# zakuro-ai/asr

Hardware: AMD Instinct MI355X
Metric: utterances/sec (10 s, 161-bin) DS2 5x1024 BiGRU CTC train step (higher is better)
Workload: dtype bf16

## Files before the change

### asr_amd/csrc/gemm_nt_w4.h

```cpp
constexpr int W4_LDS = 4 * G_TILE;
typedef __bf16 bf16x4w __attribute__((ext_vector_type(4)));
typedef float f32x2w __attribute__((ext_vector_type(2)));

__device__ __forceinline__ void w4_dma(unsigned voff, const char* sbase, unsigned lds_dst) {
  asm volatile("s_mov_b32 m0, %2\n\ts_nop 0\n\tglobal_load_lds_dwordx4 %0, %1" ::"v"(voff), "s"(sbase), "s"(lds_dst) : "memory");
}

template <bool OBF = false>
__global__ __launch_bounds__(256) void gemm_bf16_nt_w4_kernel(BArgs g, int ntx, int nty) {
  extern __shared__ __attribute__((aligned(1024))) char ldsg[];
  const int nt = ntx * nty;
  int orig = blockIdx.x;
  const int SR = g.super_rows > 0 ? g.super_rows : 1 << 20;
  auto tile_origin = [&](int o, int& tm0, int& tn0) {
    const int xcd = o & 7, q8 = nt >> 3, r8 = nt & 7;
    const int t = (xcd < r8 ? xcd * (q8 + 1) : r8 * (q8 + 1) + (xcd - r8) * q8) + (o >> 3);
    const int per = SR * ntx, sr = t / per, rem = t - sr * per;
    const int rows = min(SR, nty - sr * SR);
    const int tn = rem / rows;
    tm0 = (sr * SR + rem - tn * rows) * 256; tn0 = tn * 256;
  };
  int m0, n0;
  tile_origin(orig, m0, n0);
  const int nkt = g.K >> 6;
  const int lane = threadIdx.x & 63;
  const int wave = __builtin_amdgcn_readfirstlane(threadIdx.x >> 6);
  const int wm = wave >> 1, wn = wave & 1;
  const unsigned lds0 = (unsigned)(uintptr_t)(lds_void*)ldsg;

  unsigned voffA[8], voffB[8];
  const char* sA;
  const char* sB;
  auto retarget = [&](int tm0, int tn0) {
    int rl = lane;
    asm volatile("" : "+v"(rl));
    const int prow = rl >> 3;
#pragma unroll
    for (int p = 0; p < 8; ++p) {
      const int r = (wave + 4 * p) * 8 + prow;
      const int seg = (rl & 7) ^ ((r >> 1) & 7);
      voffA[p] = (unsigned)(min(r, g.M - 1 - tm0) * g.lda * 2 + seg * 16);
      voffB[p] = (unsigned)(min(r, g.N - 1 - tn0) * g.ldb * 2 + seg * 16);
    }
    sA = reinterpret_cast<const char*>(g.A + (long long)tm0 * g.lda);
    sB = reinterpret_cast<const char*>(g.B + (long long)tn0 * g.ldb);
  };
  retarget(m0, n0);
  const unsigned dstw = lds0 + wave * 1024;
  auto dma_a = [&](unsigned boff, int p) { w4_dma(voffA[p], sA, dstw + boff + p * 4096); };
  auto dma_b = [&](unsigned boff, int p) { w4_dma(voffB[p], sB, dstw + boff + 32768 + p * 4096); };

  const int frow = lane & 15, fseg = lane >> 4;
  const unsigned swz0 = (unsigned)((fseg ^ ((frow >> 1) & 7)) << 4);
  const unsigned raA0 = lds0 + (wm * 128 + frow) * 128 + swz0;
  const unsigned raB0 = lds0 + 32768 + (wn * 128 + frow) * 128 + swz0;

  f32x4 acc[8][8];
  f32x4 fa[2][8], fb[2][8];
#define W4_BC(x) __builtin_bit_cast(bf16x8, x)
#define W4_SB() __builtin_amdgcn_sched_barrier(0)
#define W4_RD(dst, addr, off) asm volatile("ds_read_b128 %0, %1 offset:%2" : "=v"(dst) : "v"(addr), "n"(off))
#define W4_LGKM0(F)                                                                                                                   \
  asm volatile("s_waitcnt lgkmcnt(0)"                                                                                                 \
               : "+v"(F[0]), "+v"(F[1]), "+v"(F[2]), "+v"(F[3]), "+v"(F[4]), "+v"(F[5]), "+v"(F[6]), "+v"(F[7])                       \
               :                                                                                                                      \
               : "memory")
#define W4_KTILE(DMA, VMW, NEXT)                                                                                                      \
  do {                                                                                                                                \
    const unsigned cA1 = (raA0 ^ 64u) + boff, cB1 = (raB0 ^ 64u) + boff, nA0 = raA0 + (boff ^ 65536u), nB0 = raB0 + (boff ^ 65536u);  \
    W4_SB();                                                                                                                          \
    _Pragma("unroll") for (int m_ = 0; m_ < 64; ++m_) {                                                                               \
      acc[m_ & 7][m_ >> 3] = __builtin_amdgcn_mfma_f32_16x16x32_bf16(W4_BC(fb[0][m_ >> 3]), W4_BC(fa[0][m_ & 7]), acc[m_ & 7][m_ >> 3], 0, 0, 0); \
      W4_SB();                                                                                                                        \
      if (m_ < 16 && !(m_ & 1)) W4_RD(fa[1][(m_ >> 1) & 7], cA1, ((m_ >> 1) & 7) * 2048);                                             \
      if (m_ == 19) W4_LGKM0(fa[1]);                                                                                                  \
      if (m_ == 20) __builtin_amdgcn_s_barrier();                                                                                     \
      if (m_ >= 21 && m_ <= 51 && (m_ & 1)) {                                                                                         \
        if (((m_ - 21) >> 1) & 1) W4_RD(fb[1][((m_ - 21) >> 2) & 7], cB1, (((m_ - 21) >> 2) & 7) * 2048);                             \
        else if (DMA) dma_a(boff, ((m_ - 21) >> 2) & 7);                                                                              \
      }                                                                                                                               \
      if (m_ == 54) W4_LGKM0(fb[1]);                                                                                                  \
      if (m_ == 55) __builtin_amdgcn_s_barrier();                                                                                     \
      if ((DMA) && (m_ == 57 || m_ == 59 || m_ == 61)) dma_b(boff, (m_ - 57) >> 1);                                                   \
      W4_SB();                                                                                                                        \
    }                                                                                                                                 \
    _Pragma("unroll") for (int m_ = 0; m_ < 64; ++m_) {                                                                               \
      acc[m_ & 7][m_ >> 3] = __builtin_amdgcn_mfma_f32_16x16x32_bf16(W4_BC(fb[1][m_ >> 3]), W4_BC(fa[1][m_ & 7]), acc[m_ & 7][m_ >> 3], 0, 0, 0); \
      W4_SB();                                                                                                                        \
      if ((DMA) && m_ < 10 && !(m_ & 1)) dma_b(boff, 3 + (m_ >> 1));                                                                  \
      if ((DMA) && m_ == 9) { sA += 128; sB += 128; }                                                                                 \
      if ((NEXT) && m_ == 10) asm volatile(VMW ::: "memory");                                                                         \
      if ((NEXT) && m_ == 11) __builtin_amdgcn_s_barrier();                                                                           \
      if ((NEXT) && m_ >= 13 && m_ <= 58 && (m_ - 13) % 3 == 0) {                                                                     \
        if ((m_ - 13) / 3 < 8) W4_RD(fa[0][((m_ - 13) / 3) & 7], nA0, (((m_ - 13) / 3) & 7) * 2048);                                  \
        else W4_RD(fb[0][((m_ - 13) / 3 - 8) & 7], nB0, (((m_ - 13) / 3 - 8) & 7) * 2048);                                            \
      }                                                                                                                               \
      W4_SB();                                                                                                                        \
    }                                                                                                                                 \
    if (NEXT) { W4_LGKM0(fa[0]); W4_LGKM0(fb[0]); }                                                                                   \
    W4_SB();                                                                                                                          \
    boff ^= 65536u;                                                                                                                   \
  } while (0)

  auto stage_first_two = [&]() {
#pragma unroll
    for (int p = 0; p < 8; ++p) { dma_a(0u, p); dma_b(0u, p); }
    sA += 128; sB += 128;
#pragma unroll
    for (int p = 0; p < 8; ++p) { dma_a(65536u, p); dma_b(65536u, p); }
    sA += 128; sB += 128;
  };
  stage_first_two();
  bool after_epilogue = false;
  for (;;) {
    if (after_epilogue) asm volatile("s_waitcnt vmcnt(63)" ::: "memory");
    else asm volatile("s_waitcnt vmcnt(0)" ::: "memory");
    __builtin_amdgcn_s_barrier();
    W4_SB();
#pragma unroll
    for (int i = 0; i < 8; ++i) W4_RD(fa[0][i], raA0, i * 2048);
#pragma unroll
    for (int j = 0; j < 8; ++j) W4_RD(fb[0][j], raB0, j * 2048);
#pragma unroll
    for (int i = 0; i < 8; ++i)
#pragma unroll
      for (int j = 0; j < 8; ++j) acc[i][j] = f32x4{0.f, 0.f, 0.f, 0.f};
    W4_LGKM0(fa[0]);
    W4_LGKM0(fb[0]);
    unsigned boff = 0u;
    int kt = 0;
    if (nkt > 2) {
      W4_KTILE(1, "", 1);
      kt = 1;
    }
    for (; kt < nkt - 2; ++kt) W4_KTILE(1, "s_waitcnt vmcnt(16)", 1);
    if (kt < nkt - 1) W4_KTILE(0, "s_waitcnt vmcnt(0)", 1);
    const bool more = orig + (int)gridDim.x < nt;
    int m0n = 0, n0n = 0;
    if (more) {
      tile_origin(orig + (int)gridDim.x, m0n, n0n);
      retarget(m0n, n0n);
    }
    f32x4 pbv[8];
#pragma unroll
    for (int j = 0; j < 8; ++j) {
      const int col = n0 + wn * 128 + j * 16 + fseg * 4;
      const char* bp = (g.bias && col < g.N) ? reinterpret_cast<const char*>(g.bias + col) : reinterpret_cast<const char*>(g_zero16);
      asm volatile("global_load_dwordx4 %0, %1, off" : "=v"(pbv[j]) : "v"(bp) : "memory");
    }
    W4_KTILE(0, "", 0);
    asm volatile("s_waitcnt vmcnt(0)"
                 : "+v"(pbv[0]), "+v"(pbv[1]), "+v"(pbv[2]), "+v"(pbv[3]), "+v"(pbv[4]), "+v"(pbv[5]), "+v"(pbv[6]), "+v"(pbv[7])
                 :
                 : "memory");
    if (more) stage_first_two();
    {
      float* C = g.C;
      const long long ldc = g.ldc;
      const bool stream_out = (g.nt_store & 1) != 0;
      int el = lane;
      asm volatile("" : "+v"(el));
      const int frow = el & 15, fseg = el >> 4;
      if constexpr (OBF) {
        __bf16* Cb = reinterpret_cast<__bf16*>(C);
#pragma unroll
        for (int i = 0; i < 8; ++i) {
          const int row = m0 + wm * 128 + i * 16 + frow;
#pragma unroll
          for (int j = 0; j < 8; j += 2) {
            const f32x4 va = acc[i][j] + pbv[j], vb = acc[i][j + 1] + pbv[j + 1];
            const bf16x4w pa = {(__bf16)va[0], (__bf16)va[1], (__bf16)va[2], (__bf16)va[3]};
            const bf16x4w pb = {(__bf16)vb[0], (__bf16)vb[1], (__bf16)vb[2], (__bf16)vb[3]};
            const f32x2w a2 = __builtin_bit_cast(f32x2w, pa), b2 = __builtin_bit_cast(f32x2w, pb);
            const u32pair s0 = permlane16_swap(a2[0], b2[0]), s1 = permlane16_swap(a2[1], b2[1]);
            const int col = n0 + wn * 128 + (j + (fseg & 1)) * 16 + (fseg >> 1) * 8;
            const f32x4 v = {s0.a, s1.a, s0.b, s1.b};
            f32x4* pc = (row < g.M && col < g.N) ? reinterpret_cast<f32x4*>(Cb + (long long)row * ldc + col) : reinterpret_cast<f32x4*>(g_sink16);
            if (stream_out) __builtin_nontemporal_store(v, pc);
            else *pc = v;
          }
        }
      } else
#pragma unroll
      for (int i = 0; i < 8; ++i) {
        const int row = m0 + wm * 128 + i * 16 + frow;
#pragma unroll
        for (int j = 0; j < 8; ++j) {
          const int col = n0 + wn * 128 + j * 16 + fseg * 4;
          const f32x4 v = acc[i][j] + pbv[j];
          f32x4* pc = (row < g.M && col < g.N) ? reinterpret_cast<f32x4*>(C + (long long)row * ldc + col) : reinterpret_cast<f32x4*>(g_sink16);
          if (stream_out) __builtin_nontemporal_store(v, pc);
          else *pc = v;
        }
      }
    }
    if (!more) break;
    orig += (int)gridDim.x; m0 = m0n; n0 = n0n;
    after_epilogue = true;
  }
  asm volatile("s_waitcnt vmcnt(0)" ::: "memory");
#undef W4_BC
#undef W4_SB
#undef W4_RD
#undef W4_LGKM0
#undef W4_KTILE
}
```

Measured before the change: 2828.

## Overlap previous tile's epilogue stores with next tile's first MFMA k-step

Restructures the persistent GEMM loop so the next tile's DMA staging happens continuously across tile boundaries, and the previous tile's accumulator stores (bias add plus nontemporal global stores) are interleaved into the first k-tile's MFMA stream as a 'seam' drain. Accumulators move to AGPRs via inline-asm MFMA, with a zero-C form for the first k-step, which removes explicit zeroing. Retargeting skips recomputing clamped offsets for interior tiles. The aim is to hide the epilogue store latency and the pipeline refill bubble between tiles. The cost is heavy reliance on hand-tuned waitcnt values and exec masking, which is fragile to get right.

```diff
diff --git a/asr_amd/csrc/gemm_nt_w4.h b/asr_amd/csrc/gemm_nt_w4.h
--- a/asr_amd/csrc/gemm_nt_w4.h
+++ b/asr_amd/csrc/gemm_nt_w4.h
@@ -31,16 +31,22 @@
   unsigned voffA[8], voffB[8];
   const char* sA;
   const char* sB;
+  bool clampA = true, clampB = true;
   auto retarget = [&](int tm0, int tn0) {
-    int rl = lane;
-    asm volatile("" : "+v"(rl));
-    const int prow = rl >> 3;
-#pragma unroll
-    for (int p = 0; p < 8; ++p) {
-      const int r = (wave + 4 * p) * 8 + prow;
-      const int seg = (rl & 7) ^ ((r >> 1) & 7);
-      voffA[p] = (unsigned)(min(r, g.M - 1 - tm0) * g.lda * 2 + seg * 16);
-      voffB[p] = (unsigned)(min(r, g.N - 1 - tn0) * g.ldb * 2 + seg * 16);
+    const bool eA = tm0 + 256 > g.M, eB = tn0 + 256 > g.N;
+    if (eA || clampA || eB || clampB) {
+      int rl = lane;
+      asm volatile("" : "+v"(rl));
+      const int prow = rl >> 3;
+      const int capA = (eA || clampA) ? g.M - 1 - tm0 : 255, capB = (eB || clampB) ? g.N - 1 - tn0 : 255;
+#pragma unroll
+      for (int p = 0; p < 8; ++p) {
+        const int r = (wave + 4 * p) * 8 + prow;
+        const int seg = (rl & 7) ^ ((r >> 1) & 7);
+        voffA[p] = (unsigned)(min(r, capA) * g.lda * 2 + seg * 16);
+        voffB[p] = (unsigned)(min(r, capB) * g.ldb * 2 + seg * 16);
+      }
+      clampA = eA; clampB = eB;
     }
     sA = reinterpret_cast<const char*>(g.A + (long long)tm0 * g.lda);
     sB = reinterpret_cast<const char*>(g.B + (long long)tn0 * g.ldb);
@@ -57,7 +63,6 @@
 
   f32x4 acc[8][8];
   f32x4 fa[2][8], fb[2][8];
-#define W4_BC(x) __builtin_bit_cast(bf16x8, x)
 #define W4_SB() __builtin_amdgcn_sched_barrier(0)
 #define W4_RD(dst, addr, off) asm volatile("ds_read_b128 %0, %1 offset:%2" : "=v"(dst) : "v"(addr), "n"(off))
 #define W4_LGKM0(F)                                                                                                                   \
@@ -65,30 +70,47 @@
                : "+v"(F[0]), "+v"(F[1]), "+v"(F[2]), "+v"(F[3]), "+v"(F[4]), "+v"(F[5]), "+v"(F[6]), "+v"(F[7])                       \
                :                                                                                                                      \
                : "memory")
-#define W4_KTILE(DMA, VMW, NEXT)                                                                                                      \
+#define W4_MFMA(c, b, a) asm volatile("v_mfma_f32_16x16x32_bf16 %0, %1, %2, %0" : "+a"(c) : "v"(b), "v"(a))
+#define W4_MFMA0(c, b, a) asm volatile("v_mfma_f32_16x16x32_bf16 %0, %1, %2, 0" : "+a"(c) : "v"(b), "v"(a))
+#define W4_MFMA_DONE() asm volatile("s_nop 15\n\ts_nop 7" ::: "memory")
+#define W4_ST(voff, data, sbase, imm, on)                                                                                        \
+  asm volatile("s_mov_b32 exec_lo, %4\n\ts_mov_b32 exec_hi, %4\n\tglobal_store_dwordx4 %0, %1, %2 offset:%3 nt\n\ts_mov_b64 exec, -1" \
+               ::"v"(voff), "v"(data), "s"(sbase), "n"(imm), "s"(on)                                                             \
+               : "memory")
+#define W4_KTILE(FIRST, DRAIN, VMA, VMW, NEXT)                                                                                        \
   do {                                                                                                                                \
     const unsigned cA1 = (raA0 ^ 64u) + boff, cB1 = (raB0 ^ 64u) + boff, nA0 = raA0 + (boff ^ 65536u), nB0 = raB0 + (boff ^ 65536u);  \
+    f32x4 dr_ = f32x4{0.f, 0.f, 0.f, 0.f};                                                                                            \
+    unsigned co_ = cvoff;                                                                                                             \
+    if (DRAIN) { dr_ = acc[0][0]; asm volatile("" : "+v"(dr_)); }                                                                     \
     W4_SB();                                                                                                                          \
     _Pragma("unroll") for (int m_ = 0; m_ < 64; ++m_) {                                                                               \
-      acc[m_ & 7][m_ >> 3] = __builtin_amdgcn_mfma_f32_16x16x32_bf16(W4_BC(fb[0][m_ >> 3]), W4_BC(fa[0][m_ & 7]), acc[m_ & 7][m_ >> 3], 0, 0, 0); \
-      W4_SB();                                                                                                                        \
+      if (FIRST) W4_MFMA0(acc[m_ & 7][m_ >> 3], fb[0][m_ >> 3], fa[0][m_ & 7]);                                                       \
+      else W4_MFMA(acc[m_ & 7][m_ >> 3], fb[0][m_ >> 3], fa[0][m_ & 7]);                                                              \
+      W4_SB();                                                                                                                        \
+      if (DRAIN) {                                                                                                                    \
+        const f32x4 v_ = dr_ + pbv[m_ >> 3];                                                                                          \
+        W4_ST(co_, v_, cbase, (m_ >> 3) * 64, con);                                                                                   \
+        co_ = (m_ & 7) == 7 ? cvoff : co_ + cstep;                                                                                    \
+        if (m_ < 63) { dr_ = acc[(m_ + 1) & 7][(m_ + 1) >> 3]; asm volatile("" : "+v"(dr_)); }                                        \
+      }                                                                                                                               \
       if (m_ < 16 && !(m_ & 1)) W4_RD(fa[1][(m_ >> 1) & 7], cA1, ((m_ >> 1) & 7) * 2048);                                             \
-      if (m_ == 19) W4_LGKM0(fa[1]);                                                                                                  \
+      if (m_ == 19) { asm volatile(VMA ::: "memory"); W4_LGKM0(fa[1]); }                                                              \
       if (m_ == 20) __builtin_amdgcn_s_barrier();                                                                                     \
       if (m_ >= 21 && m_ <= 51 && (m_ & 1)) {                                                                                         \
         if (((m_ - 21) >> 1) & 1) W4_RD(fb[1][((m_ - 21) >> 2) & 7], cB1, (((m_ - 21) >> 2) & 7) * 2048);                             \
-        else if (DMA) dma_a(boff, ((m_ - 21) >> 2) & 7);                                                                              \
+        else dma_a(boff, ((m_ - 21) >> 2) & 7);                                                                                       \
       }                                                                                                                               \
       if (m_ == 54) W4_LGKM0(fb[1]);                                                                                                  \
       if (m_ == 55) __builtin_amdgcn_s_barrier();                                                                                     \
-      if ((DMA) && (m_ == 57 || m_ == 59 || m_ == 61)) dma_b(boff, (m_ - 57) >> 1);                                                   \
+      if (m_ == 57 || m_ == 59 || m_ == 61) dma_b(boff, (m_ - 57) >> 1);                                                              \
       W4_SB();                                                                                                                        \
     }                                                                                                                                 \
     _Pragma("unroll") for (int m_ = 0; m_ < 64; ++m_) {                                                                               \
-      acc[m_ & 7][m_ >> 3] = __builtin_amdgcn_mfma_f32_16x16x32_bf16(W4_BC(fb[1][m_ >> 3]), W4_BC(fa[1][m_ & 7]), acc[m_ & 7][m_ >> 3], 0, 0, 0); \
-      W4_SB();                                                                                                                        \
-      if ((DMA) && m_ < 10 && !(m_ & 1)) dma_b(boff, 3 + (m_ >> 1));                                                                  \
-      if ((DMA) && m_ == 9) { sA += 128; sB += 128; }                                                                                 \
+      W4_MFMA(acc[m_ & 7][m_ >> 3], fb[1][m_ >> 3], fa[1][m_ & 7]);                                                                   \
+      W4_SB();                                                                                                                        \
+      if (m_ < 10 && !(m_ & 1)) dma_b(boff, 3 + (m_ >> 1));                                                                           \
+      if (m_ == 9) { sA += 128; sB += 128; }                                                                                          \
       if ((NEXT) && m_ == 10) asm volatile(VMW ::: "memory");                                                                         \
       if ((NEXT) && m_ == 11) __builtin_amdgcn_s_barrier();                                                                           \
       if ((NEXT) && m_ >= 13 && m_ <= 58 && (m_ - 13) % 3 == 0) {                                                                     \
@@ -102,62 +124,78 @@
     boff ^= 65536u;                                                                                                                   \
   } while (0)
 
-  auto stage_first_two = [&]() {
-#pragma unroll
-    for (int p = 0; p < 8; ++p) { dma_a(0u, p); dma_b(0u, p); }
-    sA += 128; sB += 128;
-#pragma unroll
-    for (int p = 0; p < 8; ++p) { dma_a(65536u, p); dma_b(65536u, p); }
-    sA += 128; sB += 128;
+#pragma unroll
+  for (int p = 0; p < 8; ++p) { dma_a(0u, p); dma_b(0u, p); }
+  sA += 128; sB += 128;
+#pragma unroll
+  for (int p = 0; p < 8; ++p) { dma_a(65536u, p); dma_b(65536u, p); }
+  sA += 128; sB += 128;
+  asm volatile("s_waitcnt vmcnt(0)" ::: "memory");
+#pragma unroll
+  for (int i = 0; i < 8; ++i)
+#pragma unroll
+    for (int j = 0; j < 8; ++j) asm volatile("" : "=a"(acc[i][j]));
+  unsigned boff = 0u;
+
+  const bool stream_out = (g.nt_store & 1) != 0;
+  bool more = false;
+  int m0n = 0, n0n = 0;
+  auto stage_next_tile = [&]() {
+    more = orig + (int)gridDim.x < nt;
+    m0n = m0; n0n = n0;
+    if (more) tile_origin(orig + (int)gridDim.x, m0n, n0n);
+    retarget(m0n, n0n);
   };
-  stage_first_two();
-  bool after_epilogue = false;
+  bool drain = false;
+  int mo = 0, no = 0;
+  f32x4 pbv[8] = {};
+  unsigned cvoff = 0u, cstep = 0u;
+  const char* cbase = nullptr;
+  int con = 0;
   for (;;) {
-    if (after_epilogue) asm volatile("s_waitcnt vmcnt(63)" ::: "memory");
-    else asm volatile("s_waitcnt vmcnt(0)" ::: "memory");
     __builtin_amdgcn_s_barrier();
     W4_SB();
 #pragma unroll
-    for (int i = 0; i < 8; ++i) W4_RD(fa[0][i], raA0, i * 2048);
-#pragma unroll
-    for (int j = 0; j < 8; ++j) W4_RD(fb[0][j], raB0, j * 2048);
-#pragma unroll
-    for (int i = 0; i < 8; ++i)
-#pragma unroll
-      for (int j = 0; j < 8; ++j) acc[i][j] = f32x4{0.f, 0.f, 0.f, 0.f};
+    for (int i = 0; i < 8; ++i) W4_RD(fa[0][i], raA0 + boff, i * 2048);
+#pragma unroll
+    for (int j = 0; j < 8; ++j) W4_RD(fb[0][j], raB0 + boff, j * 2048);
     W4_LGKM0(fa[0]);
     W4_LGKM0(fb[0]);
-    unsigned boff = 0u;
-    int kt = 0;
-    if (nkt > 2) {
-      W4_KTILE(1, "", 1);
-      kt = 1;
-    }
-    for (; kt < nkt - 2; ++kt) W4_KTILE(1, "s_waitcnt vmcnt(16)", 1);
-    if (kt < nkt - 1) W4_KTILE(0, "s_waitcnt vmcnt(0)", 1);
-    const bool more = orig + (int)gridDim.x < nt;
-    int m0n = 0, n0n = 0;
-    if (more) {
-      tile_origin(orig + (int)gridDim.x, m0n, n0n);
-      retarget(m0n, n0n);
-    }
-    f32x4 pbv[8];
+    W4_SB();
+    if (nkt == 2) stage_next_tile();
+    if constexpr (OBF) {
+      W4_KTILE(1, 0, "", "", 1);
+    } else {
+      if (drain) {
+        int el = lane;
+        asm volatile("" : "+v"(el));
+        cvoff = (unsigned)(((el & 15) * g.ldc + (el >> 4) * 4) * 4);
+        cstep = (unsigned)(g.ldc * 64);
+        cbase = reinterpret_cast<const char*>(g.C + (long long)(mo + wm * 128) * g.ldc + no + wn * 128);
+      }
+      con = __builtin_amdgcn_readfirstlane(drain ? -1 : 0);
+      W4_KTILE(1, 1, "s_waitcnt vmcnt(20)", "", 1);
+    }
+    for (int kt = 1; kt < nkt - 1; ++kt) {
+      if (kt == nkt - 2) stage_next_tile();
+      W4_KTILE(0, 0, "", "s_waitcnt vmcnt(16)", 1);
+    }
+    const bool seam = !OBF && more && stream_out && m0 + 256 <= g.M && n0 + 256 <= g.N && g.ldc < (1 << 22);
 #pragma unroll
     for (int j = 0; j < 8; ++j) {
       const int col = n0 + wn * 128 + j * 16 + fseg * 4;
       const char* bp = (g.bias && col < g.N) ? reinterpret_cast<const char*>(g.bias + col) : reinterpret_cast<const char*>(g_zero16);
       asm volatile("global_load_dwordx4 %0, %1, off" : "=v"(pbv[j]) : "v"(bp) : "memory");
     }
-    W4_KTILE(0, "", 0);
-    asm volatile("s_waitcnt vmcnt(0)"
+    W4_KTILE(0, 0, "", "", 0);
+    W4_MFMA_DONE();
+    asm volatile("s_waitcnt vmcnt(16)"
                  : "+v"(pbv[0]), "+v"(pbv[1]), "+v"(pbv[2]), "+v"(pbv[3]), "+v"(pbv[4]), "+v"(pbv[5]), "+v"(pbv[6]), "+v"(pbv[7])
                  :
                  : "memory");
-    if (more) stage_first_two();
-    {
+    if (!seam) {
       float* C = g.C;
       const long long ldc = g.ldc;
-      const bool stream_out = (g.nt_store & 1) != 0;
       int el = lane;
       asm volatile("" : "+v"(el));
       const int frow = el & 15, fseg = el >> 4;
@@ -179,6 +217,7 @@
             if (stream_out) __builtin_nontemporal_store(v, pc);
             else *pc = v;
           }
+          W4_SB();
         }
       } else
 #pragma unroll
@@ -187,19 +226,27 @@
 #pragma unroll
         for (int j = 0; j < 8; ++j) {
           const int col = n0 + wn * 128 + j * 16 + fseg * 4;
-          const f32x4 v = acc[i][j] + pbv[j];
+          f32x4 t = acc[i][j];
+          asm volatile("" : "+v"(t));
+          const f32x4 v = t + pbv[j];
           f32x4* pc = (row < g.M && col < g.N) ? reinterpret_cast<f32x4*>(C + (long long)row * ldc + col) : reinterpret_cast<f32x4*>(g_sink16);
           if (stream_out) __builtin_nontemporal_store(v, pc);
           else *pc = v;
         }
+        W4_SB();
       }
+      if constexpr (OBF) asm volatile("s_waitcnt vmcnt(32)" ::: "memory");
+      else asm volatile("s_waitcnt vmcnt(63)" ::: "memory");
     }
     if (!more) break;
+    drain = seam; mo = m0; no = n0;
     orig += (int)gridDim.x; m0 = m0n; n0 = n0n;
-    after_epilogue = true;
   }
   asm volatile("s_waitcnt vmcnt(0)" ::: "memory");
-#undef W4_BC
+#undef W4_ST
+#undef W4_MFMA
+#undef W4_MFMA0
+#undef W4_MFMA_DONE
 #undef W4_SB
 #undef W4_RD
 #undef W4_LGKM0
```

After: 2827. Within noise of the previous version (-0.0%).
